# Cornell-RelaxML/QuIP

Hardware: NVIDIA H100
Metric: tokens/sec 2-bit Llama-2-7B (per-layer eval path, seq 2048) (higher is better)
Workload: dtype f16

## Files before the change

quip_b200/csrc/qgemm_tc.cu:

```cuda
#include "tc_common.cuh"

namespace quip {

constexpr int TC_SMEM_MAX = 227 * 1024;

template <int BITS, int BN, bool DENSE>
struct TcCfg {
  static constexpr int A_BYTES = DENSE ? TC_BM * TC_BK * 2 : (TC_BM / SB_ROWS) * sb_words(BITS) * 4;
  static constexpr int B_BYTES = BN * TC_BK * 2;
  static constexpr int STAGE_BYTES = A_BYTES + B_BYTES;
  static constexpr int EPI_HALVES = BN * 72 > 64 * (BN + 8) ? BN * 72 : 64 * (BN + 8);
  static constexpr int EPI_BYTES = 2 * EPI_HALVES * 2;
  static constexpr int STAGES_FIT = (TC_SMEM_MAX - EPI_BYTES - 1024 - 256) / STAGE_BYTES;
  static constexpr int STAGES = STAGES_FIT < 16 ? STAGES_FIT : 16;
  static constexpr size_t SMEM = (size_t)STAGES * STAGE_BYTES + 1024  + 256  + EPI_BYTES;
  static_assert(STAGE_BYTES % 1024 == 0 && 2 * STAGES * 8 <= 256, "stage layout");
};

template <int BITS, int BN, bool DENSE>
__global__ void __launch_bounds__(TC_THREADS, 1)
qgemm_tc_kernel(const __grid_constant__ CUtensorMap tmap_x, const __grid_constant__ CUtensorMap tmap_a,
                const float* __restrict__ scales, const float* __restrict__ zeros, const __half* __restrict__ bias,
                const float* __restrict__ xsum, __half* __restrict__ z, int M, int K, int N, int symmetric, int nblk,
                int shared_factor) {
  using C = TcCfg<BITS, BN, DENSE>;
  extern __shared__ unsigned char smem_raw[];
  const uint32_t smem_base = (smem_u32(smem_raw) + 1023u) & ~1023u;
  unsigned char* smem_gen = smem_raw + (smem_base - smem_u32(smem_raw));
  uint64_t* bars = reinterpret_cast<uint64_t*>(smem_gen + (size_t)C::STAGES * C::STAGE_BYTES);
  uint64_t* full = bars;
  uint64_t* empty = bars + C::STAGES;
  __half* epi = reinterpret_cast<__half*>(smem_gen + (size_t)C::STAGES * C::STAGE_BYTES + 256);

  const int warp = threadIdx.x >> 5, lane = threadIdx.x & 31;
  const int tiles_n = DENSE ? (N + BN - 1) / BN : (N + TC_BM - 1) / TC_BM;
  const int tiles_m = DENSE ? (M + TC_BM - 1) / TC_BM : (M + BN - 1) / BN;
  const int per_blk = tiles_n * tiles_m;
  const int num_tiles = per_blk * nblk;
  const int KB = (K + TC_BK - 1) / TC_BK;
  const int64_t ldz = (int64_t)N * nblk;
  constexpr int TMA_WARP = TC_CONSUMER_WARPS;

  if (warp == TMA_WARP && lane == 0) {
    asm volatile("prefetch.tensormap [%0];" ::"l"(&tmap_x) : "memory");
    asm volatile("prefetch.tensormap [%0];" ::"l"(&tmap_a) : "memory");
    for (int s = 0; s < C::STAGES; ++s) {
      mbar_init(&full[s], 1);
      mbar_init(&empty[s], TC_CONSUMER_WARPS);
    }
    asm volatile("fence.mbarrier_init.release.cluster;" ::: "memory");
  }
  __syncthreads();

  if (warp == TMA_WARP) {
    if (lane == 0) {
      int s = 0;
      uint32_t ph = 0;
      for (int tile = blockIdx.x; tile < num_tiles; tile += gridDim.x) {
        const int blk = tile / per_blk, rr = tile % per_blk;
        const int m0 = (rr / tiles_n) * (DENSE ? TC_BM : BN), n0 = (rr % tiles_n) * (DENSE ? BN : TC_BM);
        for (int kb = 0; kb < KB; ++kb) {
          mbar_wait(&empty[s], ph ^ 1u);
          unsigned char* stage = smem_gen + (size_t)s * C::STAGE_BYTES;
          if (DENSE) {
            mbar_arrive_expect_tx(&full[s], C::STAGE_BYTES);
            tma_load_2d(stage, &tmap_x, &full[s], blk * K + kb * TC_BK, m0);
            tma_load_3d(stage + C::A_BYTES, &tmap_a, &full[s], kb * TC_BK, n0, shared_factor ? 0 : blk);
          } else {
            const bool words = (kb & 1) == 0;
            mbar_arrive_expect_tx(&full[s], C::B_BYTES + (words ? C::A_BYTES : 0));
            if (words) tma_load_2d(stage, &tmap_a, &full[s], (kb >> 1) * sb_words(BITS), n0 / SB_ROWS);
            tma_load_2d(stage + C::A_BYTES, &tmap_x, &full[s], kb * TC_BK, m0);
          }
          if (++s == C::STAGES) { s = 0; ph ^= 1u; }
        }
      }
    }
  } else {
    const int wg = warp >> 2, wtid = threadIdx.x & 127;
    const int frow = (warp & 3) * 16 + (lane >> 2);
    const int fcol = (lane & 3) * 2;
    __half* eb = epi + wg * C::EPI_HALVES;
    float acc[BN / 2];
#pragma unroll
    for (int j = 0; j < BN / 2; ++j) acc[j] = 0.f;
    int s = 0;
    uint32_t ph = 0;
    auto advance = [&]() { if (++s == C::STAGES) { s = 0; ph ^= 1u; } };
    auto release = [&](int st) {
      __syncwarp();
      if (lane == 0) mbar_arrive(&empty[st]);
    };
    for (int tile = blockIdx.x; tile < num_tiles; tile += gridDim.x) {
      const int blk = tile / per_blk, rr = tile % per_blk;
      int prev = 0;
      const int n_base = (rr % tiles_n) * TC_BM + wg * 64, m0 = (rr / tiles_n) * BN;
      float Pn[2], Rn[2], bn[2];
      if constexpr (!DENSE) {
#pragma unroll
        for (int h = 0; h < 2; ++h) {
          const int n = n_base + frow + 8 * h;
          Pn[h] = 1.f; Rn[h] = 0.f; bn[h] = 0.f;
          if (n < N) {
            const float sc = scales[n];
            Pn[h] = sc * (float)(1 << BITS);
            if (!symmetric) Rn[h] = sc * (0.5f * (float)((1 << BITS) - 1)) - zeros[n];
            if (bias) bn[h] = __half2float(bias[n]);
          }
        }
        if (!symmetric && wtid < BN / 32 && m0 + 32 * wtid < M)
          asm volatile("prefetch.global.L1 [%0];" ::"l"(xsum + m0 + 32 * wtid));
      }
      if constexpr (DENSE) {
        for (int kb = 0; kb < KB; ++kb) {
          mbar_wait(&full[s], ph);
          const uint32_t a_addr = smem_base + (uint32_t)(s * C::STAGE_BYTES);
          const uint64_t adesc = make_sw128_desc(a_addr + (uint32_t)(wg * 64 * 128));
          const uint64_t bdesc = make_sw128_desc(a_addr + C::A_BYTES);
          wgmma_fence();
#pragma unroll
          for (int k = 0; k < TC_BK / 16; ++k)
            wgmma_f16_ss<BN>(acc, adesc + (uint64_t)(2 * k), bdesc + (uint64_t)(2 * k), (kb | k) ? 1 : 0);
          wgmma_commit();
          wgmma_wait<1>();
          if (kb > 0) release(prev);
          prev = s;
          advance();
        }
      } else {
        const int g = lane >> 2, t = lane & 3;
        const uint32_t row_off = (uint32_t)(warp * sb_words(BITS) * 4);
        uint32_t w[row_words(BITS)];
        uint32_t fa[2][16];
        auto issue = [&](const uint32_t (&f)[16], int first) {
          const uint64_t bdesc = make_sw128_desc(smem_base + (uint32_t)(s * C::STAGE_BYTES) + C::A_BYTES);
          wgmma_fence();
#pragma unroll
          for (int k = 0; k < TC_BK / 16; ++k)
            wgmma_f16_rs<BN>(acc, &f[4 * k], bdesc + (uint64_t)(2 * k), (first && k == 0) ? 0 : 1);
          wgmma_commit();
        };
        auto load_words = [&]() {
          mbar_wait(&full[s], ph);
          tc_load_row_words<BITS>(smem_base + (uint32_t)(s * C::STAGE_BYTES) + row_off, g, w);
        };
        load_words();
        frag_natural<BITS, 0, 0>(w, t, &fa[0][0]);
        frag_natural<BITS, 0, 1>(w, t, &fa[0][4]);
        frag_natural<BITS, 1, 0>(w, t, &fa[0][8]);
        frag_natural<BITS, 1, 1>(w, t, &fa[0][12]);
        const int KSB = KB >> 1;
        for (int ksb = 0; ksb < KSB; ++ksb) {
          const int se = s;
          issue(fa[0], ksb == 0);
          wgmma_wait<1>();
          if (ksb > 0) release(prev);
          advance();
          mbar_wait(&full[s], ph);
          frag_natural<BITS, 2, 0>(w, t, &fa[1][0]);
          frag_natural<BITS, 2, 1>(w, t, &fa[1][4]);
          frag_natural<BITS, 3, 0>(w, t, &fa[1][8]);
          frag_natural<BITS, 3, 1>(w, t, &fa[1][12]);
          issue(fa[1], 0);
          wgmma_wait<1>();
          release(se);
          prev = s;
          advance();
          if (ksb + 1 < KSB) {
            load_words();
            frag_natural<BITS, 0, 0>(w, t, &fa[0][0]);
            frag_natural<BITS, 0, 1>(w, t, &fa[0][4]);
            frag_natural<BITS, 1, 0>(w, t, &fa[0][8]);
            frag_natural<BITS, 1, 1>(w, t, &fa[0][12]);
          }
        }
      }
      wgmma_wait<0>();
      wgmma_fence_regs(acc);
      release(prev);

      if constexpr (DENSE) {
        constexpr int EP = BN + 8;
#pragma unroll
        for (int j = 0; j < BN / 2; j += 2) {
          const int r = frow + ((j & 2) ? 8 : 0), c = 8 * (j >> 2) + fcol;
          *reinterpret_cast<__half2*>(&eb[r * EP + c]) = __floats2half2_rn(acc[j], acc[j + 1]);
        }
        asm volatile("bar.sync %0, 128;" ::"r"(1 + wg) : "memory");
        const int m_base = (rr / tiles_n) * TC_BM + wg * 64, i0 = (rr % tiles_n) * BN;
        for (int idx = wtid; idx < 64 * (BN / 8); idx += 128) {
          const int r = idx / (BN / 8), v = idx % (BN / 8);
          const int m = m_base + r, i = i0 + 8 * v;
          if (m < M && i < N)
            *reinterpret_cast<uint4*>(z + (int64_t)m * ldz + (int64_t)blk * N + i) =
                *reinterpret_cast<const uint4*>(&eb[r * EP + 8 * v]);
        }
      } else {
        constexpr int EP = 72;
#pragma unroll
        for (int j = 0; j < BN / 2; ++j) {
          const int h = (j >> 1) & 1, c = 8 * (j >> 2) + fcol + (j & 1), m = m0 + c;
          float v = Pn[h] * acc[j] + bn[h];
          if (!symmetric) v += Rn[h] * (m < M ? __ldg(&xsum[m]) : 0.f);
          eb[c * EP + frow + 8 * h] = __float2half_rn(v);
        }
        asm volatile("bar.sync %0, 128;" ::"r"(1 + wg) : "memory");
        for (int idx = wtid; idx < BN * 8; idx += 128) {
          const int c = idx >> 3, v = idx & 7;
          const int m = m0 + c, n = n_base + 8 * v;
          if (m < M && n < N)
            *reinterpret_cast<uint4*>(z + (int64_t)m * ldz + n) = *reinterpret_cast<const uint4*>(&eb[c * EP + 8 * v]);
        }
      }
      asm volatile("bar.sync %0, 128;" ::"r"(1 + wg) : "memory");
    }
  }
}

typedef CUresult (*PFN_encodeTiled)(CUtensorMap*, CUtensorMapDataType, cuuint32_t, void*, const cuuint64_t*,
                                    const cuuint64_t*, const cuuint32_t*, const cuuint32_t*, CUtensorMapInterleave,
                                    CUtensorMapSwizzle, CUtensorMapL2promotion, CUtensorMapFloatOOBfill);

static PFN_encodeTiled get_encode() {
  static PFN_encodeTiled fn = nullptr;
  if (!fn) {
    void* p = nullptr;
    cudaDriverEntryPointQueryResult qres;
    if (cudaGetDriverEntryPoint("cuTensorMapEncodeTiled", &p, cudaEnableDefault, &qres) == cudaSuccess &&
        qres == cudaDriverEntryPointSuccess)
      fn = (PFN_encodeTiled)p;
  }
  return fn;
}

static int g_num_sms = 0;

int num_sms() {
  if (!g_num_sms) {
    int dev = 0;
    if (cudaGetDevice(&dev) != cudaSuccess ||
        cudaDeviceGetAttribute(&g_num_sms, cudaDevAttrMultiProcessorCount, dev) != cudaSuccess)
      g_num_sms = 132;
  }
  return g_num_sms;
}

int make_act_map(CUtensorMap* tmap, const void* x, int64_t rows, int64_t cols, int box_rows) {
  PFN_encodeTiled enc = get_encode();
  if (!enc) {
    set_error("cuTensorMapEncodeTiled is not available from the driver");
    return QUIP_ERR_CUDA;
  }
  cuuint64_t dims[2] = {(cuuint64_t)cols, (cuuint64_t)rows};
  cuuint64_t strides[1] = {(cuuint64_t)cols * sizeof(__half)};
  cuuint32_t box[2] = {(cuuint32_t)TC_BK, (cuuint32_t)box_rows};
  cuuint32_t estr[2] = {1, 1};
  CUresult r = enc(tmap, CU_TENSOR_MAP_DATA_TYPE_FLOAT16, 2, (void*)x, dims, strides, box, estr,
                   CU_TENSOR_MAP_INTERLEAVE_NONE, CU_TENSOR_MAP_SWIZZLE_128B, CU_TENSOR_MAP_L2_PROMOTION_L2_256B,
                   CU_TENSOR_MAP_FLOAT_OOB_FILL_NONE);
  if (r != CUDA_SUCCESS) {
    set_error("cuTensorMapEncodeTiled failed with CUresult %d (ptr=%p rows=%lld cols=%lld)", (int)r, x,
              (long long)rows, (long long)cols);
    return QUIP_ERR_CUDA;
  }
  return QUIP_OK;
}

static int make_words_map(CUtensorMap* tmap, const QuipLinearDesc* d) {
  PFN_encodeTiled enc = get_encode();
  if (!enc) {
    set_error("cuTensorMapEncodeTiled is not available from the driver");
    return QUIP_ERR_CUDA;
  }
  const int sbw = sb_words(d->bits);
  cuuint64_t dims[2] = {(cuuint64_t)(d->K / SB_K) * sbw, (cuuint64_t)(d->N / SB_ROWS)};
  cuuint64_t strides[1] = {dims[0] * sizeof(uint32_t)};
  cuuint32_t box[2] = {(cuuint32_t)sbw, (cuuint32_t)(TC_BM / SB_ROWS)};
  cuuint32_t estr[2] = {1, 1};
  CUresult r = enc(tmap, CU_TENSOR_MAP_DATA_TYPE_UINT32, 2, (void*)d->qweight, dims, strides, box, estr,
                   CU_TENSOR_MAP_INTERLEAVE_NONE, CU_TENSOR_MAP_SWIZZLE_NONE, CU_TENSOR_MAP_L2_PROMOTION_L2_256B,
                   CU_TENSOR_MAP_FLOAT_OOB_FILL_NONE);
  if (r != CUDA_SUCCESS) {
    set_error("cuTensorMapEncodeTiled (packed words) failed with CUresult %d (N=%d K=%d bits=%d)", (int)r, d->N, d->K,
              d->bits);
    return QUIP_ERR_CUDA;
  }
  return QUIP_OK;
}

template <int BITS, int BN>
static int launch_tc(const QuipLinearDesc* d, const __half* x, const float* xsum, const __half* bias, __half* z,
                     int M, cudaStream_t s) {
  using C = TcCfg<BITS, BN, false>;
  CUtensorMap tmx, tmq;
  if (int e = make_act_map(&tmx, x, M, d->K, BN)) return e;
  if (int e = make_words_map(&tmq, d)) return e;
  auto kern = qgemm_tc_kernel<BITS, BN, false>;
  QUIP_CUDA(cudaFuncSetAttribute(kern, cudaFuncAttributeMaxDynamicSharedMemorySize, (int)C::SMEM));
  int tiles = ceil_div(d->N, TC_BM) * ceil_div(M, BN);
  int grid = tiles < num_sms() ? tiles : num_sms();
  kern<<<grid, TC_THREADS, C::SMEM, s>>>(tmx, tmq, d->scales, d->zeros, bias, xsum, z, M, d->K, d->N,
                                         (d->flags & QUIP_FLAG_SYMMETRIC) ? 1 : 0, 1, 0);
  QUIP_LAUNCHED("qgemm_tc_kernel");
  return QUIP_OK;
}

template <int BN>
static int launch_tc_dense(const QuipPass* ps, const __half* in, __half* out, int M, int n, cudaStream_t s) {
  using C = TcCfg<2, BN, true>;
  PFN_encodeTiled enc = get_encode();
  CUtensorMap tmx, tma;
  if (int e = make_act_map(&tmx, in, M, n, TC_BM)) return e;
  const int p = ps->p;
  cuuint64_t dims[3] = {(cuuint64_t)p, (cuuint64_t)p, (cuuint64_t)(ps->shared ? 1 : ps->nblk)};
  cuuint64_t strides[2] = {(cuuint64_t)p * sizeof(__half), (cuuint64_t)p * p * sizeof(__half)};
  cuuint32_t box[3] = {(cuuint32_t)TC_BK, (cuuint32_t)BN, 1};
  cuuint32_t estr[3] = {1, 1, 1};
  CUresult r = enc(&tma, CU_TENSOR_MAP_DATA_TYPE_FLOAT16, 3, (void*)ps->factors, dims, strides, box, estr,
                   CU_TENSOR_MAP_INTERLEAVE_NONE, CU_TENSOR_MAP_SWIZZLE_128B, CU_TENSOR_MAP_L2_PROMOTION_L2_256B,
                   CU_TENSOR_MAP_FLOAT_OOB_FILL_NONE);
  if (r != CUDA_SUCCESS) {
    set_error("cuTensorMapEncodeTiled (factors) failed with CUresult %d (p=%d nblk=%d)", (int)r, p, ps->nblk);
    return QUIP_ERR_CUDA;
  }
  auto kern = qgemm_tc_kernel<2, BN, true>;
  QUIP_CUDA(cudaFuncSetAttribute(kern, cudaFuncAttributeMaxDynamicSharedMemorySize, (int)C::SMEM));
  int tiles = ceil_div(p, BN) * ceil_div(M, TC_BM) * ps->nblk;
  int grid = tiles < num_sms() ? tiles : num_sms();
  kern<<<grid, TC_THREADS, C::SMEM, s>>>(tmx, tma, nullptr, nullptr, nullptr, nullptr, out, M, p, p, 1,
                                         ps->nblk, ps->shared ? 1 : 0);
  QUIP_LAUNCHED("qgemm_tc_kernel<dense>");
  return QUIP_OK;
}

int pass_big_tc(const QuipPass* ps, const __half* in, __half* out, int64_t M, int n, cudaStream_t s) {
  QUIP_CHECK_ARG(!ps->strided && ps->p % 8 == 0 && n % 8 == 0, "tensor-core pass needs contiguous blocks, p %% 8 == 0");
  QUIP_CHECK_ARG((((uintptr_t)in | (uintptr_t)out | (uintptr_t)ps->factors) & 15) == 0, "tensor-core pass: unaligned pointer");
  return launch_tc_dense<128>(ps, in, out, (int)M, n, s);
}

int qgemm_tc(const QuipLinearDesc* d, const __half* x, const float* xsum, const __half* bias, __half* z, int M,
             cudaStream_t s) {
  QUIP_CHECK_ARG((((uintptr_t)x | (uintptr_t)d->qweight) & 15) == 0,
                 "tensor-core path needs 16-byte aligned activations and packed words");
  const bool wide = M > 64;
#define QUIP_TC(B)                                                            \
  if (d->bits == B)                                                           \
    return wide ? launch_tc<B, 128>(d, x, xsum, bias, z, M, s) : launch_tc<B, 64>(d, x, xsum, bias, z, M, s);
  QUIP_TC(2) QUIP_TC(3) QUIP_TC(4)
#undef QUIP_TC
  set_error("tensor-core kernel: unsupported bits=%d", d->bits);
  return QUIP_ERR_UNSUPPORTED;
}

}
```

quip_b200/csrc/tc_common.cuh:

```cuda
#pragma once
#include <cuda.h>

#include "common.cuh"

namespace quip {

constexpr int TC_BM = 128;
constexpr int TC_BK = 64;
constexpr int TC_CONSUMER_WARPS = 8;
constexpr int TC_THREADS = 32 * TC_CONSUMER_WARPS + 32;
constexpr uint32_t TC_WATCHDOG = 1u << 28;

__device__ __forceinline__ void mbar_init(uint64_t* bar, uint32_t count) {
  asm volatile("mbarrier.init.shared::cta.b64 [%0], %1;" ::"r"(smem_u32(bar)), "r"(count));
}
__device__ __forceinline__ void mbar_wait(uint64_t* bar, uint32_t parity) {
  uint32_t addr = smem_u32(bar), done = 0, spins = 0;
  while (true) {
    asm volatile(
        "{\n\t.reg .pred p;\n\t"
        "mbarrier.try_wait.parity.shared::cta.b64 p, [%1], %2;\n\t"
        "selp.u32 %0, 1, 0, p;\n\t}"
        : "=r"(done)
        : "r"(addr), "r"(parity)
        : "memory");
    if (done) break;
    if (++spins > TC_WATCHDOG) __trap();
  }
}
__device__ __forceinline__ void mbar_arrive(uint64_t* bar) {
  asm volatile("mbarrier.arrive.shared::cta.b64 _, [%0];" ::"r"(smem_u32(bar)) : "memory");
}
__device__ __forceinline__ void mbar_arrive_expect_tx(uint64_t* bar, uint32_t bytes) {
  asm volatile("mbarrier.arrive.expect_tx.shared::cta.b64 _, [%0], %1;" ::"r"(smem_u32(bar)), "r"(bytes) : "memory");
}
__device__ __forceinline__ void tma_load_2d(void* smem_dst, const CUtensorMap* map, uint64_t* bar, int c0, int c1) {
  asm volatile(
      "cp.async.bulk.tensor.2d.shared::cluster.global.mbarrier::complete_tx::bytes [%0], [%1, {%3, %4}], [%2];"
      ::"r"(smem_u32(smem_dst)), "l"(map), "r"(smem_u32(bar)), "r"(c0), "r"(c1)
      : "memory");
}
__device__ __forceinline__ void tma_load_3d(void* smem_dst, const CUtensorMap* map, uint64_t* bar, int c0, int c1, int c2) {
  asm volatile(
      "cp.async.bulk.tensor.3d.shared::cluster.global.mbarrier::complete_tx::bytes [%0], [%1, {%3, %4, %5}], [%2];"
      ::"r"(smem_u32(smem_dst)), "l"(map), "r"(smem_u32(bar)), "r"(c0), "r"(c1), "r"(c2)
      : "memory");
}

__device__ __forceinline__ uint64_t make_sw128_desc(uint32_t smem_addr) {
  uint64_t d = 0;
  d |= (uint64_t)((smem_addr & 0x3FFFFu) >> 4);
  d |= (uint64_t)1 << 16;
  d |= (uint64_t)(1024 >> 4) << 32;
  d |= (uint64_t)1 << 62;
  return d;
}

template <int N>
__device__ __forceinline__ void wgmma_f16_ss(float (&d)[N / 2], uint64_t adesc, uint64_t bdesc, int scale_d);
template <>
__device__ __forceinline__ void wgmma_f16_ss<64>(float (&d)[32], uint64_t adesc, uint64_t bdesc, int scale_d) {
  asm volatile(
      "{\n\t.reg .pred p;\n\t"
      "setp.ne.b32 p, %34, 0;\n\t"
      "wgmma.mma_async.sync.aligned.m64n64k16.f32.f16.f16 "
      "{%0,%1,%2,%3,%4,%5,%6,%7,%8,%9,%10,%11,%12,%13,%14,%15,%16,%17,%18,%19,%20,%21,%22,%23,%24,%25,%26,%27,%28,%29,%30,%31}, "
      "%32, %33, p, 1, 1, 0, 0;\n\t}"
      : "+f"(d[0]), "+f"(d[1]), "+f"(d[2]), "+f"(d[3]), "+f"(d[4]), "+f"(d[5]), "+f"(d[6]), "+f"(d[7]), "+f"(d[8]), "+f"(d[9]), "+f"(d[10]), "+f"(d[11]), "+f"(d[12]), "+f"(d[13]), "+f"(d[14]), "+f"(d[15]), "+f"(d[16]), "+f"(d[17]), "+f"(d[18]), "+f"(d[19]), "+f"(d[20]), "+f"(d[21]), "+f"(d[22]), "+f"(d[23]), "+f"(d[24]), "+f"(d[25]), "+f"(d[26]), "+f"(d[27]), "+f"(d[28]), "+f"(d[29]), "+f"(d[30]), "+f"(d[31])
      : "l"(adesc), "l"(bdesc), "r"(scale_d));
}

template <>
__device__ __forceinline__ void wgmma_f16_ss<128>(float (&d)[64], uint64_t adesc, uint64_t bdesc, int scale_d) {
  asm volatile(
      "{\n\t.reg .pred p;\n\t"
      "setp.ne.b32 p, %66, 0;\n\t"
      "wgmma.mma_async.sync.aligned.m64n128k16.f32.f16.f16 "
      "{%0,%1,%2,%3,%4,%5,%6,%7,%8,%9,%10,%11,%12,%13,%14,%15,%16,%17,%18,%19,%20,%21,%22,%23,%24,%25,%26,%27,%28,%29,%30,%31,%32,%33,%34,%35,%36,%37,%38,%39,%40,%41,%42,%43,%44,%45,%46,%47,%48,%49,%50,%51,%52,%53,%54,%55,%56,%57,%58,%59,%60,%61,%62,%63}, "
      "%64, %65, p, 1, 1, 0, 0;\n\t}"
      : "+f"(d[0]), "+f"(d[1]), "+f"(d[2]), "+f"(d[3]), "+f"(d[4]), "+f"(d[5]), "+f"(d[6]), "+f"(d[7]), "+f"(d[8]), "+f"(d[9]), "+f"(d[10]), "+f"(d[11]), "+f"(d[12]), "+f"(d[13]), "+f"(d[14]), "+f"(d[15]), "+f"(d[16]), "+f"(d[17]), "+f"(d[18]), "+f"(d[19]), "+f"(d[20]), "+f"(d[21]), "+f"(d[22]), "+f"(d[23]), "+f"(d[24]), "+f"(d[25]), "+f"(d[26]), "+f"(d[27]), "+f"(d[28]), "+f"(d[29]), "+f"(d[30]), "+f"(d[31]), "+f"(d[32]), "+f"(d[33]), "+f"(d[34]), "+f"(d[35]), "+f"(d[36]), "+f"(d[37]), "+f"(d[38]), "+f"(d[39]), "+f"(d[40]), "+f"(d[41]), "+f"(d[42]), "+f"(d[43]), "+f"(d[44]), "+f"(d[45]), "+f"(d[46]), "+f"(d[47]), "+f"(d[48]), "+f"(d[49]), "+f"(d[50]), "+f"(d[51]), "+f"(d[52]), "+f"(d[53]), "+f"(d[54]), "+f"(d[55]), "+f"(d[56]), "+f"(d[57]), "+f"(d[58]), "+f"(d[59]), "+f"(d[60]), "+f"(d[61]), "+f"(d[62]), "+f"(d[63])
      : "l"(adesc), "l"(bdesc), "r"(scale_d));
}
__device__ __forceinline__ void wgmma_fence() { asm volatile("wgmma.fence.sync.aligned;" ::: "memory"); }
__device__ __forceinline__ void wgmma_commit() { asm volatile("wgmma.commit_group.sync.aligned;" ::: "memory"); }
template <int PENDING>
__device__ __forceinline__ void wgmma_wait() { asm volatile("wgmma.wait_group.sync.aligned %0;" ::"n"(PENDING) : "memory"); }
template <int R>
__device__ __forceinline__ void wgmma_fence_regs(float (&d)[R]) {
#pragma unroll
  for (int i = 0; i < R; ++i) asm volatile("" : "+f"(d[i])::"memory");
}

template <int N>
__device__ __forceinline__ void wgmma_f16_rs(float (&d)[N / 2], const uint32_t* a, uint64_t bdesc, int scale_d);
template <>
__device__ __forceinline__ void wgmma_f16_rs<64>(float (&d)[32], const uint32_t* a, uint64_t bdesc, int scale_d) {
  asm volatile(
      "{\n\t.reg .pred p;\n\t"
      "setp.ne.b32 p, %37, 0;\n\t"
      "wgmma.mma_async.sync.aligned.m64n64k16.f32.f16.f16 "
      "{%0,%1,%2,%3,%4,%5,%6,%7,%8,%9,%10,%11,%12,%13,%14,%15,%16,%17,%18,%19,%20,%21,%22,%23,%24,%25,%26,%27,%28,%29,%30,%31}, "
      "{%32,%33,%34,%35}, %36, p, 1, 1, 0;\n\t}"
      : "+f"(d[0]), "+f"(d[1]), "+f"(d[2]), "+f"(d[3]), "+f"(d[4]), "+f"(d[5]), "+f"(d[6]), "+f"(d[7]), "+f"(d[8]), "+f"(d[9]), "+f"(d[10]), "+f"(d[11]), "+f"(d[12]), "+f"(d[13]), "+f"(d[14]), "+f"(d[15]), "+f"(d[16]), "+f"(d[17]), "+f"(d[18]), "+f"(d[19]), "+f"(d[20]), "+f"(d[21]), "+f"(d[22]), "+f"(d[23]), "+f"(d[24]), "+f"(d[25]), "+f"(d[26]), "+f"(d[27]), "+f"(d[28]), "+f"(d[29]), "+f"(d[30]), "+f"(d[31])
      : "r"(a[0]), "r"(a[1]), "r"(a[2]), "r"(a[3]), "l"(bdesc), "r"(scale_d));
}
template <>
__device__ __forceinline__ void wgmma_f16_rs<128>(float (&d)[64], const uint32_t* a, uint64_t bdesc, int scale_d) {
  asm volatile(
      "{\n\t.reg .pred p;\n\t"
      "setp.ne.b32 p, %69, 0;\n\t"
      "wgmma.mma_async.sync.aligned.m64n128k16.f32.f16.f16 "
      "{%0,%1,%2,%3,%4,%5,%6,%7,%8,%9,%10,%11,%12,%13,%14,%15,%16,%17,%18,%19,%20,%21,%22,%23,%24,%25,%26,%27,%28,%29,%30,%31,%32,%33,%34,%35,%36,%37,%38,%39,%40,%41,%42,%43,%44,%45,%46,%47,%48,%49,%50,%51,%52,%53,%54,%55,%56,%57,%58,%59,%60,%61,%62,%63}, "
      "{%64,%65,%66,%67}, %68, p, 1, 1, 0;\n\t}"
      : "+f"(d[0]), "+f"(d[1]), "+f"(d[2]), "+f"(d[3]), "+f"(d[4]), "+f"(d[5]), "+f"(d[6]), "+f"(d[7]), "+f"(d[8]), "+f"(d[9]), "+f"(d[10]), "+f"(d[11]), "+f"(d[12]), "+f"(d[13]), "+f"(d[14]), "+f"(d[15]), "+f"(d[16]), "+f"(d[17]), "+f"(d[18]), "+f"(d[19]), "+f"(d[20]), "+f"(d[21]), "+f"(d[22]), "+f"(d[23]), "+f"(d[24]), "+f"(d[25]), "+f"(d[26]), "+f"(d[27]), "+f"(d[28]), "+f"(d[29]), "+f"(d[30]), "+f"(d[31]), "+f"(d[32]), "+f"(d[33]), "+f"(d[34]), "+f"(d[35]), "+f"(d[36]), "+f"(d[37]), "+f"(d[38]), "+f"(d[39]), "+f"(d[40]), "+f"(d[41]), "+f"(d[42]), "+f"(d[43]), "+f"(d[44]), "+f"(d[45]), "+f"(d[46]), "+f"(d[47]), "+f"(d[48]), "+f"(d[49]), "+f"(d[50]), "+f"(d[51]), "+f"(d[52]), "+f"(d[53]), "+f"(d[54]), "+f"(d[55]), "+f"(d[56]), "+f"(d[57]), "+f"(d[58]), "+f"(d[59]), "+f"(d[60]), "+f"(d[61]), "+f"(d[62]), "+f"(d[63])
      : "r"(a[0]), "r"(a[1]), "r"(a[2]), "r"(a[3]), "l"(bdesc), "r"(scale_d));
}

template <int BITS>
__device__ __forceinline__ void tc_load_row_words(uint32_t rb, int g, uint32_t (&w)[row_words(BITS)]) {
  auto ld4 = [](uint32_t addr, uint32_t* d) {
    asm volatile("ld.shared.v4.b32 {%0,%1,%2,%3}, [%4];" : "=r"(d[0]), "=r"(d[1]), "=r"(d[2]), "=r"(d[3]) : "r"(addr));
  };
#pragma unroll
  for (int i = 0; i < 4; ++i) ld4(rb + (uint32_t)(16 * g + 4 * i) * 4u, &w[4 * i]);
  if constexpr (BITS == 3) {
#pragma unroll
    for (int i = 0; i < 2; ++i) ld4(rb + (uint32_t)(128 + 8 * g + 4 * i) * 4u, &w[16 + 4 * i]);
  } else if constexpr (BITS == 4) {
#pragma unroll
    for (int i = 0; i < 4; ++i) ld4(rb + (uint32_t)(128 + 16 * g + 4 * i) * 4u, &w[16 + 4 * i]);
  }
}
}
```

Baseline: 19570.

## Write GEMM epilogue via stmatrix into swizzled smem and TMA bulk stores

```diff
diff --git a/quip_b200/csrc/qgemm_tc.cu b/quip_b200/csrc/qgemm_tc.cu
--- a/quip_b200/csrc/qgemm_tc.cu
+++ b/quip_b200/csrc/qgemm_tc.cu
@@ -9,28 +9,27 @@
   static constexpr int A_BYTES = DENSE ? TC_BM * TC_BK * 2 : (TC_BM / SB_ROWS) * sb_words(BITS) * 4;
   static constexpr int B_BYTES = BN * TC_BK * 2;
   static constexpr int STAGE_BYTES = A_BYTES + B_BYTES;
-  static constexpr int EPI_HALVES = BN * 72 > 64 * (BN + 8) ? BN * 72 : 64 * (BN + 8);
-  static constexpr int EPI_BYTES = 2 * EPI_HALVES * 2;
-  static constexpr int STAGES_FIT = (TC_SMEM_MAX - EPI_BYTES - 1024 - 256) / STAGE_BYTES;
+  static constexpr int OUT_BYTES = BN * 64 * 2;
+  static constexpr int STAGES_FIT = (TC_SMEM_MAX - 2 * OUT_BYTES - 1024 - 256) / STAGE_BYTES;
   static constexpr int STAGES = STAGES_FIT < 16 ? STAGES_FIT : 16;
-  static constexpr size_t SMEM = (size_t)STAGES * STAGE_BYTES + 1024  + 256  + EPI_BYTES;
-  static_assert(STAGE_BYTES % 1024 == 0 && 2 * STAGES * 8 <= 256, "stage layout");
+  static constexpr size_t SMEM = (size_t)STAGES * STAGE_BYTES + 2 * OUT_BYTES + 1024  + 256 ;
+  static_assert(STAGE_BYTES % 1024 == 0 && OUT_BYTES % 1024 == 0 && 2 * STAGES * 8 <= 256, "stage layout");
 };
 
 template <int BITS, int BN, bool DENSE>
 __global__ void __launch_bounds__(TC_THREADS, 1)
 qgemm_tc_kernel(const __grid_constant__ CUtensorMap tmap_x, const __grid_constant__ CUtensorMap tmap_a,
-                const float* __restrict__ scales, const float* __restrict__ zeros, const __half* __restrict__ bias,
-                const float* __restrict__ xsum, __half* __restrict__ z, int M, int K, int N, int symmetric, int nblk,
-                int shared_factor) {
+                const __grid_constant__ CUtensorMap tmap_z, const float* __restrict__ scales,
+                const float* __restrict__ zeros, const __half* __restrict__ bias, const float* __restrict__ xsum,
+                int M, int K, int N, int symmetric, int nblk, int shared_factor) {
   using C = TcCfg<BITS, BN, DENSE>;
   extern __shared__ unsigned char smem_raw[];
   const uint32_t smem_base = (smem_u32(smem_raw) + 1023u) & ~1023u;
   unsigned char* smem_gen = smem_raw + (smem_base - smem_u32(smem_raw));
-  uint64_t* bars = reinterpret_cast<uint64_t*>(smem_gen + (size_t)C::STAGES * C::STAGE_BYTES);
+  const uint32_t out_base = smem_base + (uint32_t)(C::STAGES * C::STAGE_BYTES);
+  uint64_t* bars = reinterpret_cast<uint64_t*>(smem_gen + (size_t)C::STAGES * C::STAGE_BYTES + 2 * C::OUT_BYTES);
   uint64_t* full = bars;
   uint64_t* empty = bars + C::STAGES;
-  __half* epi = reinterpret_cast<__half*>(smem_gen + (size_t)C::STAGES * C::STAGE_BYTES + 256);
 
   const int warp = threadIdx.x >> 5, lane = threadIdx.x & 31;
   const int tiles_n = DENSE ? (N + BN - 1) / BN : (N + TC_BM - 1) / TC_BM;
@@ -38,12 +37,12 @@
   const int per_blk = tiles_n * tiles_m;
   const int num_tiles = per_blk * nblk;
   const int KB = (K + TC_BK - 1) / TC_BK;
-  const int64_t ldz = (int64_t)N * nblk;
   constexpr int TMA_WARP = TC_CONSUMER_WARPS;
 
   if (warp == TMA_WARP && lane == 0) {
     asm volatile("prefetch.tensormap [%0];" ::"l"(&tmap_x) : "memory");
     asm volatile("prefetch.tensormap [%0];" ::"l"(&tmap_a) : "memory");
+    asm volatile("prefetch.tensormap [%0];" ::"l"(&tmap_z) : "memory");
     for (int s = 0; s < C::STAGES; ++s) {
       mbar_init(&full[s], 1);
       mbar_init(&empty[s], TC_CONSUMER_WARPS);
@@ -80,7 +79,7 @@
     const int wg = warp >> 2, wtid = threadIdx.x & 127;
     const int frow = (warp & 3) * 16 + (lane >> 2);
     const int fcol = (lane & 3) * 2;
-    __half* eb = epi + wg * C::EPI_HALVES;
+    const uint32_t ob = out_base + (uint32_t)(wg * C::OUT_BYTES);
     float acc[BN / 2];
 #pragma unroll
     for (int j = 0; j < BN / 2; ++j) acc[j] = 0.f;
@@ -179,41 +178,54 @@
       wgmma_fence_regs(acc);
       release(prev);
 
+      const int q = lane >> 3, r8 = lane & 7;
+      if (wtid == 0) bulk_wait_read_all();
+      asm volatile("bar.sync %0, 128;" ::"r"(1 + wg) : "memory");
       if constexpr (DENSE) {
-        constexpr int EP = BN + 8;
-#pragma unroll
-        for (int j = 0; j < BN / 2; j += 2) {
-          const int r = frow + ((j & 2) ? 8 : 0), c = 8 * (j >> 2) + fcol;
-          *reinterpret_cast<__half2*>(&eb[r * EP + c]) = __floats2half2_rn(acc[j], acc[j + 1]);
-        }
-        asm volatile("bar.sync %0, 128;" ::"r"(1 + wg) : "memory");
-        const int m_base = (rr / tiles_n) * TC_BM + wg * 64, i0 = (rr % tiles_n) * BN;
-        for (int idx = wtid; idx < 64 * (BN / 8); idx += 128) {
-          const int r = idx / (BN / 8), v = idx % (BN / 8);
-          const int m = m_base + r, i = i0 + 8 * v;
-          if (m < M && i < N)
-            *reinterpret_cast<uint4*>(z + (int64_t)m * ldz + (int64_t)blk * N + i) =
-                *reinterpret_cast<const uint4*>(&eb[r * EP + 8 * v]);
+#pragma unroll
+        for (int j0 = 0; j0 < BN / 2; j0 += 8) {
+          const uint32_t f[4] = {pack_half2_rn(acc[j0], acc[j0 + 1]), pack_half2_rn(acc[j0 + 2], acc[j0 + 3]),
+                                 pack_half2_rn(acc[j0 + 4], acc[j0 + 5]), pack_half2_rn(acc[j0 + 6], acc[j0 + 7])};
+          const int cg = (j0 >> 2) + (q >> 1), row = (warp & 3) * 16 + 8 * (q & 1) + r8;
+          stmatrix_x4(ob + (uint32_t)((cg >> 3) * 64 * 128 + row * 128 + (((cg & 7) ^ r8) << 4)), f);
         }
       } else {
-        constexpr int EP = 72;
-#pragma unroll
-        for (int j = 0; j < BN / 2; ++j) {
-          const int h = (j >> 1) & 1, c = 8 * (j >> 2) + fcol + (j & 1), m = m0 + c;
-          float v = Pn[h] * acc[j] + bn[h];
-          if (!symmetric) v += Rn[h] * (m < M ? __ldg(&xsum[m]) : 0.f);
-          eb[c * EP + frow + 8 * h] = __float2half_rn(v);
-        }
-        asm volatile("bar.sync %0, 128;" ::"r"(1 + wg) : "memory");
-        for (int idx = wtid; idx < BN * 8; idx += 128) {
-          const int c = idx >> 3, v = idx & 7;
-          const int m = m0 + c, n = n_base + 8 * v;
-          if (m < M && n < N)
-            *reinterpret_cast<uint4*>(z + (int64_t)m * ldz + n) = *reinterpret_cast<const uint4*>(&eb[c * EP + 8 * v]);
-        }
-      }
+#pragma unroll
+        for (int j0 = 0; j0 < BN / 2; j0 += 8) {
+          uint32_t f[4];
+#pragma unroll
+          for (int u = 0; u < 4; ++u) {
+            float v2[2];
+#pragma unroll
+            for (int e = 0; e < 2; ++e) {
+              const int j = j0 + 2 * u + e;
+              const int h = (j >> 1) & 1, c = 8 * (j >> 2) + fcol + (j & 1), m = m0 + c;
+              float v = Pn[h] * acc[j] + bn[h];
+              if (!symmetric) v += Rn[h] * (m < M ? __ldg(&xsum[m]) : 0.f);
+              v2[e] = v;
+            }
+            f[u] = pack_half2_rn(v2[0], v2[1]);
+          }
+          const int row = 8 * ((j0 >> 2) + (q >> 1)) + r8, chunk = 2 * (warp & 3) + (q & 1);
+          stmatrix_x4_trans(ob + (uint32_t)(row * 128 + ((chunk ^ r8) << 4)), f);
+        }
+      }
+      fence_proxy_async_smem();
       asm volatile("bar.sync %0, 128;" ::"r"(1 + wg) : "memory");
+      if (wtid == 0) {
+        if constexpr (DENSE) {
+          const int m_base = (rr / tiles_n) * TC_BM + wg * 64, i0 = (rr % tiles_n) * BN;
+#pragma unroll
+          for (int half = 0; half < BN / 64; ++half)
+            if (m_base < M && i0 + 64 * half < N)
+              tma_store_3d(ob + (uint32_t)(half * 64 * 128), &tmap_z, i0 + 64 * half, blk, m_base);
+        } else {
+          if (n_base < N) tma_store_2d(ob, &tmap_z, n_base, m0);
+        }
+        bulk_commit();
+      }
     }
+    if (wtid == 0) bulk_wait_all();
   }
 }
 
@@ -292,14 +304,15 @@
 static int launch_tc(const QuipLinearDesc* d, const __half* x, const float* xsum, const __half* bias, __half* z,
                      int M, cudaStream_t s) {
   using C = TcCfg<BITS, BN, false>;
-  CUtensorMap tmx, tmq;
+  CUtensorMap tmx, tmq, tmz;
   if (int e = make_act_map(&tmx, x, M, d->K, BN)) return e;
   if (int e = make_words_map(&tmq, d)) return e;
+  if (int e = make_act_map(&tmz, z, M, d->N, BN)) return e;
   auto kern = qgemm_tc_kernel<BITS, BN, false>;
   QUIP_CUDA(cudaFuncSetAttribute(kern, cudaFuncAttributeMaxDynamicSharedMemorySize, (int)C::SMEM));
   int tiles = ceil_div(d->N, TC_BM) * ceil_div(M, BN);
   int grid = tiles < num_sms() ? tiles : num_sms();
-  kern<<<grid, TC_THREADS, C::SMEM, s>>>(tmx, tmq, d->scales, d->zeros, bias, xsum, z, M, d->K, d->N,
+  kern<<<grid, TC_THREADS, C::SMEM, s>>>(tmx, tmq, tmz, d->scales, d->zeros, bias, xsum, M, d->K, d->N,
                                          (d->flags & QUIP_FLAG_SYMMETRIC) ? 1 : 0, 1, 0);
   QUIP_LAUNCHED("qgemm_tc_kernel");
   return QUIP_OK;
@@ -323,12 +336,22 @@
     set_error("cuTensorMapEncodeTiled (factors) failed with CUresult %d (p=%d nblk=%d)", (int)r, p, ps->nblk);
     return QUIP_ERR_CUDA;
   }
+  CUtensorMap tmz;
+  cuuint64_t zdims[3] = {(cuuint64_t)p, (cuuint64_t)ps->nblk, (cuuint64_t)M};
+  cuuint64_t zstrides[2] = {(cuuint64_t)p * sizeof(__half), (cuuint64_t)p * ps->nblk * sizeof(__half)};
+  cuuint32_t zbox[3] = {64, 1, 64};
+  r = enc(&tmz, CU_TENSOR_MAP_DATA_TYPE_FLOAT16, 3, (void*)out, zdims, zstrides, zbox, estr, CU_TENSOR_MAP_INTERLEAVE_NONE,
+          CU_TENSOR_MAP_SWIZZLE_128B, CU_TENSOR_MAP_L2_PROMOTION_NONE, CU_TENSOR_MAP_FLOAT_OOB_FILL_NONE);
+  if (r != CUDA_SUCCESS) {
+    set_error("cuTensorMapEncodeTiled (pass output) failed with CUresult %d (p=%d nblk=%d M=%d)", (int)r, p, ps->nblk, M);
+    return QUIP_ERR_CUDA;
+  }
   auto kern = qgemm_tc_kernel<2, BN, true>;
   QUIP_CUDA(cudaFuncSetAttribute(kern, cudaFuncAttributeMaxDynamicSharedMemorySize, (int)C::SMEM));
   int tiles = ceil_div(p, BN) * ceil_div(M, TC_BM) * ps->nblk;
   int grid = tiles < num_sms() ? tiles : num_sms();
-  kern<<<grid, TC_THREADS, C::SMEM, s>>>(tmx, tma, nullptr, nullptr, nullptr, nullptr, out, M, p, p, 1,
-                                         ps->nblk, ps->shared ? 1 : 0);
+  kern<<<grid, TC_THREADS, C::SMEM, s>>>(tmx, tma, tmz, nullptr, nullptr, nullptr, nullptr, M, p, p, 1, ps->nblk,
+                                         ps->shared ? 1 : 0);
   QUIP_LAUNCHED("qgemm_tc_kernel<dense>");
   return QUIP_OK;
 }
@@ -341,8 +364,8 @@
 
 int qgemm_tc(const QuipLinearDesc* d, const __half* x, const float* xsum, const __half* bias, __half* z, int M,
              cudaStream_t s) {
-  QUIP_CHECK_ARG((((uintptr_t)x | (uintptr_t)d->qweight) & 15) == 0,
-                 "tensor-core path needs 16-byte aligned activations and packed words");
+  QUIP_CHECK_ARG((((uintptr_t)x | (uintptr_t)d->qweight | (uintptr_t)z) & 15) == 0,
+                 "tensor-core path needs 16-byte aligned activations, packed words and output");
   const bool wide = M > 64;
 #define QUIP_TC(B)                                                            \
   if (d->bits == B)                                                           \
diff --git a/quip_b200/csrc/tc_common.cuh b/quip_b200/csrc/tc_common.cuh
--- a/quip_b200/csrc/tc_common.cuh
+++ b/quip_b200/csrc/tc_common.cuh
@@ -46,6 +46,33 @@
       ::"r"(smem_u32(smem_dst)), "l"(map), "r"(smem_u32(bar)), "r"(c0), "r"(c1), "r"(c2)
       : "memory");
 }
+
+__device__ __forceinline__ void stmatrix_x4(uint32_t addr, const uint32_t (&r)[4]) {
+  asm volatile("stmatrix.sync.aligned.m8n8.x4.shared.b16 [%0], {%1, %2, %3, %4};"
+               ::"r"(addr), "r"(r[0]), "r"(r[1]), "r"(r[2]), "r"(r[3]) : "memory");
+}
+__device__ __forceinline__ void stmatrix_x4_trans(uint32_t addr, const uint32_t (&r)[4]) {
+  asm volatile("stmatrix.sync.aligned.m8n8.x4.trans.shared.b16 [%0], {%1, %2, %3, %4};"
+               ::"r"(addr), "r"(r[0]), "r"(r[1]), "r"(r[2]), "r"(r[3]) : "memory");
+}
+__device__ __forceinline__ uint32_t pack_half2_rn(float lo, float hi) {
+  __half2 h = __floats2half2_rn(lo, hi);
+  return *reinterpret_cast<uint32_t*>(&h);
+}
+__device__ __forceinline__ void fence_proxy_async_smem() {
+  asm volatile("fence.proxy.async.shared::cta;" ::: "memory");
+}
+__device__ __forceinline__ void tma_store_2d(uint32_t smem_src, const CUtensorMap* map, int c0, int c1) {
+  asm volatile("cp.async.bulk.tensor.2d.global.shared::cta.bulk_group [%0, {%2, %3}], [%1];"
+               ::"l"(map), "r"(smem_src), "r"(c0), "r"(c1) : "memory");
+}
+__device__ __forceinline__ void tma_store_3d(uint32_t smem_src, const CUtensorMap* map, int c0, int c1, int c2) {
+  asm volatile("cp.async.bulk.tensor.3d.global.shared::cta.bulk_group [%0, {%2, %3, %4}], [%1];"
+               ::"l"(map), "r"(smem_src), "r"(c0), "r"(c1), "r"(c2) : "memory");
+}
+__device__ __forceinline__ void bulk_commit() { asm volatile("cp.async.bulk.commit_group;" ::: "memory"); }
+__device__ __forceinline__ void bulk_wait_read_all() { asm volatile("cp.async.bulk.wait_group.read 0;" ::: "memory"); }
+__device__ __forceinline__ void bulk_wait_all() { asm volatile("cp.async.bulk.wait_group 0;" ::: "memory"); }
 
 __device__ __forceinline__ uint64_t make_sw128_desc(uint32_t smem_addr) {
   uint64_t d = 0;
```

Result: no change. 19600 (median of 6 runs) (+0.2%).
